# tnestmeyer/reflectance-filtering

Hardware: AMD Instinct MI355X
Metric: megapixels/sec joint-bilateral sigma_c=20 sigma_s=22 @1080p (higher is better)
Workload: dtype f32

## Files before the change

### reflectance_filtering_amd/csrc/rf_api.hip

```cpp
#include "rf_common.hpp"

#include <atomic>
#include <cstring>

#include "reflectance_filtering_debug.h"

namespace rf {

void jbf_shutdown();
void cnn_shutdown();
void gf_shutdown();

char *last_error_buf()
{
    static thread_local char buf[512] = "";
    return buf;
}

int fail(int code, const char *fmt, ...)
{
    va_list ap;
    va_start(ap, fmt);
    vsnprintf(last_error_buf(), 512, fmt, ap);
    va_end(ap);
    return code;
}

static std::atomic<int> g_debug[kDbgCount];

int debug_get(int id) { return g_debug[id].load(std::memory_order_relaxed); }

}

extern "C" int rf_debug_option(const char *name, int value)
{
    static const char *const names[] = {"gf_two_kernel",     "jbf_stage_only",
                                                      "jbf_compiler_loop", "jbf_tile64_only",
                                                      "jbf_tune",          "jbf_f32_untiled",
                                                      "cnn_lds_columns",   "gf_seg_rows",
                                                      "gf_one_stream",     "gf_force_two_streams",
                                                      "gf_guide_cache",    "gf_chained",        "gf_no_compact",
                                                      "gf_exp_skip",       "gf_stagger",        "gf_parts",
                                                      "gf_s1_cap",         "gf_s1_min_wgs",
                                                      "jbf_lookahead1",    "gf_s1_legacy_strips",
                                                      "gf_exact_all_flagged", "gf_cw_chan_run",   "gf_exact",
                                                      "jbf_no_msad",       "colorize_chunk_px"};
    static_assert(sizeof(names) / sizeof(names[0]) == rf::kDbgCount, "one name per DebugOption");
    if (name)
        for (int i = 0; i < rf::kDbgCount; i++)
            if (std::strcmp(name, names[i]) == 0)
                return rf::g_debug[i].exchange(value < 0 ? 0 : value);
    return rf::fail(RF_E_BADARG, "rf_debug_option: unknown option '%s'", name ? name : "(null)");
}

__global__ void clock_probe_kernel(unsigned long long *out, unsigned long long ticks)
{
    if (threadIdx.x != 0)
        return;
    const unsigned long long r0 = __builtin_amdgcn_s_memrealtime();
    const unsigned long long c0 = __builtin_amdgcn_s_memtime();
    unsigned long long r1 = r0;
    while (r1 - r0 < ticks) {
        __builtin_amdgcn_s_sleep(64);
        r1 = __builtin_amdgcn_s_memrealtime();
    }
    const unsigned long long c1 = __builtin_amdgcn_s_memtime();
    r1 = __builtin_amdgcn_s_memrealtime();
    out[0] = c1 - c0;
    out[1] = r1 - r0;
}

extern "C" int rf_debug_clock_probe(unsigned long long *out2, int micros, void *stream)
{
    if (!out2 || micros < 1 || micros > 1000000)
        return rf::fail(RF_E_BADARG, "rf_debug_clock_probe: bad argument");
    hipLaunchKernelGGL(clock_probe_kernel, dim3(1), dim3(64), 0, (hipStream_t)stream, out2,
                       (unsigned long long)micros * 100ull);
    RF_HIP_CHECK(hipGetLastError());
    return RF_OK;
}

#ifdef RF_GF_DEV_ONLY
extern "C" int rf_version(void) { return RF_VERSION | 0x40000000; }
#else
extern "C" int rf_version(void) { return RF_VERSION; }
#endif

#ifndef RF_TOOLCHAIN
#define RF_TOOLCHAIN "unknown toolchain"
#endif
extern "C" const char *rf_debug_build_info(void) { return RF_TOOLCHAIN; }

extern "C" const char *rf_last_error(void) { return rf::last_error_buf(); }

extern "C" int rf_shutdown(void)
{
    rf::jbf_shutdown();
    rf::cnn_shutdown();
    rf::gf_shutdown();
// ... 3 lines not shown
```

### reflectance_filtering_amd/csrc/rf_common.hpp

```cpp
#pragma once
#include <hip/hip_runtime.h>

#include <cstdarg>
#include <cstdint>
#include <cstdio>

#include "reflectance_filtering.h"

namespace rf {

char *last_error_buf();
int fail(int code, const char *fmt, ...);

#define RF_HIP_CHECK(expr)                                                                   \
    do {                                                                                     \
        hipError_t _e = (expr);                                                              \
        if (_e != hipSuccess)                                                                \
            return ::rf::fail(RF_E_HIP, "%s failed: %s (%s:%d)", #expr, hipGetErrorString(_e), \
                              __FILE__, __LINE__);                                           \
    } while (0)

__host__ __device__ inline int border_interpolate(int p, int len, int border)
{
    if ((unsigned)p < (unsigned)len)
// ... 22 lines not shown
__device__ inline uint8_t saturate_u8(float v)
{
    if (!(fabsf(v) < 2147483648.0f))
        return 0;
    int iv = __float2int_rn(v);
    iv = iv < 0 ? 0 : (iv > 255 ? 255 : iv);
    return (uint8_t)iv;
}

inline int ceil_div(int a, int b) { return (a + b - 1) / b; }

inline bool ranges_overlap(const void *a, size_t na, const void *b, size_t nb)
{
    const uintptr_t a0 = (uintptr_t)a, b0 = (uintptr_t)b;
    return a0 < b0 + nb && b0 < a0 + na;
}

inline bool stream_is_capturing(hipStream_t stream)
{
    hipStreamCaptureStatus cs = hipStreamCaptureStatusNone;
    if (hipStreamIsCapturing(stream, &cs) != hipSuccess) {
        (void)hipGetLastError();
        return false;
    }
    return cs != hipStreamCaptureStatusNone;
}

enum DebugOption {
    kDbgGfTwoKernel = 0,
    kDbgJbfStageOnly,
    kDbgJbfCompilerLoop,
    kDbgJbfTile64Only,
    kDbgJbfTune,
    kDbgJbfF32Untiled,
    kDbgCnnLdsColumns,
    kDbgGfSegRows,
    kDbgGfOneStream,
    kDbgGfForceTwoStreams,
    kDbgGfGuideCache,
    kDbgGfChained,
    kDbgGfNoCompact,
    kDbgGfExpSkip,
    kDbgGfStagger,
    kDbgGfParts,
    kDbgGfS1Cap,
    kDbgGfS1MinWgs,
    kDbgJbfLookahead1,
    kDbgGfS1LegacyStrips,
    kDbgGfExactAllFlagged,
    kDbgGfCwChanRun,
    kDbgGfExact,
    kDbgJbfNoMsad,
    kDbgColorizeChunkPx,
    kDbgCount
};
int debug_get(int id);

}
```

### reflectance_filtering_amd/csrc/rf_jbf.hip

```cpp
#include <algorithm>
#include <mutex>
#include <vector>

#include "rf_jbf_common.hpp"
#include "rf_jbf_tables.hpp"
#include "rf_jbf_taploops.hpp"

namespace rf {
namespace {

constexpr int kTileW = 64;
constexpr int kMaxLds = 160 * 1024;
constexpr int kTlw2 = 144;
constexpr int kJbfMaxTiledR4 = 468;
constexpr int kJbfStageOnly = 0x1000, kJbfCompilerLoop = 0x2000, kJbfTile64Only = 0x4000;
constexpr int kJbfLookahead1 = 0x8000;
constexpr int kJbfNoMsad = 0x10000;

int jbf_debug_flags()
{
    return (debug_get(kDbgJbfStageOnly) ? kJbfStageOnly : 0) |
           (debug_get(kDbgJbfCompilerLoop) ? kJbfCompilerLoop : 0) |
           (debug_get(kDbgJbfTile64Only) ? kJbfTile64Only : 0) |
           (debug_get(kDbgJbfLookahead1) ? kJbfLookahead1 : 0) |
// ... 212 lines not shown
        const int X = 4 * tx + p + r4;
        jc[p] = tile[(ty + radius) * TLW + (X & 3) * Q4 + (X >> 2)].x;
    }
    const uint32_t lut_lane_addr = lds_addr(lutrep) + lane_lut * 4u;
    const uint32_t sw_addr0 = lds_addr(swl);
    const uint32_t tile_lane_addr = lds_addr(tile) + (uint32_t)tx * 8u;

    float sum[kPix][SCN];
    float wsum[kPix];
#pragma unroll
    for (int p = 0; p < kPix; p++) {
        wsum[p] = 0.f;
#pragma unroll
        for (int c = 0; c < SCN; c++)
            sum[p][c] = 0.f;
    }
    if (SCN == 3 && !all_grey) {
        jbf_tap_loop<SCN, LUTREP, CLAMP, TLW, 8>(lut_lane_addr, sw_addr0, tile_lane_addr, 0u, jc, amax,
                                              ty, radius, r4, sw_len, hwtab, sum, wsum);
    } else {
        float sum1[kPix][1];
#pragma unroll
        for (int p = 0; p < kPix; p++)
            sum1[p][0] = 0.f;
        jbf_tap_loop<1, LUTREP, CLAMP, TLW, 8>(lut_lane_addr, sw_addr0, tile_lane_addr, 0u, jc, amax, ty,
                                            radius, r4, sw_len, hwtab, sum1, wsum);
#pragma unroll
        for (int p = 0; p < kPix; p++)
#pragma unroll
            for (int c = 0; c < SCN; c++)
                sum[p][c] = sum1[p][0];
    }

    store_quad<SCN, SCN>(dst, img, tile_y0 + ty, tile_x0 + 4 * tx, h, w, sum, wsum, flags);
}

constexpr int kT64Lds = 163840;

struct alignas(16) JbfTileRec {
    unsigned long long first;
    int h, w, tile_y0, tile_x0, pad[2];
};
static_assert(sizeof(JbfTileRec) == 32, "the workspace holds 32 bytes per tile");

template <bool kRagged>
struct JbfTilesArg {
    using type = int;
};
template <>
struct JbfTilesArg<true> {
    using type = const JbfTileRec *__restrict__;
};

template <int SCN, int GREP, int CREP, int TLW, int TH = 64, bool kRagged = false>
__global__ __launch_bounds__(1024) void jbf_tile64_kernel(
    const uint8_t *__restrict__ joint, const uint8_t *__restrict__ src, uint8_t *__restrict__ dst,
    int h, int w, int jcn, int radius, int border, const float *__restrict__ lut, int nz,
    const int *__restrict__ hwtab, const float *__restrict__ swsym, int sw_len,
    typename JbfTilesArg<kRagged>::type tiles_x, int tiles_per_img, int flags, int crows, int y_base,
    int x_base)
{
    constexpr int NT = 1024;
    constexpr int QW = NT / TH;
    constexpr int TW = 4 * QW;
    static_assert(TH == 64 || TH == 32 || ((TH == 16 || TH == 128) && SCN == 1), "tile shapes");
    static_assert(QW >= 32 || (QW == 16 && TLW % 32 == 16) || (QW == 8 && TLW % 32 == 8),
                  "row pitch keeps the rows of a half-wave on disjoint banks");
    constexpr int Q4 = TLW / 4;
    extern __shared__ __align__(16) unsigned char smem[];
    volatile int *flag_word = reinterpret_cast<volatile int *>(smem);
    const bool need_sw = (flags & (kJbfCompilerLoop | kJbfLookahead1)) != 0;
    float *swl = reinterpret_cast<float *>(smem + 16);
    const int sw_bytes = need_sw ? ((radius + 1) * sw_len * 4 + 15) & ~15 : 0;
    unsigned char *tile_raw = smem + 16 + sw_bytes;
    if (threadIdx.x == 0)
        *flag_word = 3;
    __syncthreads();

    const int tid = threadIdx.x;
    const int tile_id = xcd_contiguous_tile((int)blockIdx.x, (int)gridDim.x);
    int tile_y0, tile_x0;
    size_t img;
    if constexpr (kRagged) {
        const JbfTileRec *rec = tiles_x + tile_id;
        img = (size_t)rec->first;
        h = rec->h;
        w = rec->w;
        tile_y0 = rec->tile_y0;
        tile_x0 = rec->tile_x0;
    } else {
        const int img_idx = tile_id / tiles_per_img;
        const int t_in_img = tile_id - img_idx * tiles_per_img;
        tile_y0 = y_base + (t_in_img / tiles_x) * TH;
        tile_x0 = x_base + (t_in_img % tiles_x) * TW;
        img = (size_t)img_idx * h * w;
    }
    const int r4 = (radius + 3) & ~3;
    const int tx = tid % QW;
    const int ty = tid / QW;

    if (need_sw)
        for (int i = tid; i < (radius + 1) * sw_len; i += NT)
            swl[i] = swsym[i];
    float *lut_g = reinterpret_cast<float *>(smem + kT64Lds - nz * GREP * 4);
    for (int i = tid; i < nz * GREP; i += NT)
        lut_g[i] = lut[i / GREP];
    uint32_t *tile4 = reinterpret_cast<uint32_t *>(tile_raw);
    int grey = 1, grey_joint = 1;
    const bool j1_ok = !(flags & kJbfCompilerLoop);
    const bool j1 = SCN == 1 && jcn != 3 && j1_ok;
    const uint32_t j1_scale = (uint32_t)(jcn == 1 ? 1 : 3) * (GREP * 4u);
    const int tlh = TH + 2 * radius;
    for (int item = tid; item < tlh * Q4; item += NT) {
        const int ry = item / Q4, k = item - ry * Q4;
        const int gy = border_interpolate(tile_y0 - radius + ry, h, border);
        uint32_t jv[4], sv[4];
        load_tile_quad(joint, src, img, gy, tile_x0 - r4 + 4 * k, w, jcn, SCN, border, jv, sv);
#pragma unroll
        for (int u = 0; u < 4; u++) {
            if (SCN == 3)
                grey &= (int)(((sv[u] ^ (sv[u] >> 8)) & 0xffffu) == 0u);
            if (jcn == 3)
                grey_joint &= (int)(((jv[u] ^ (jv[u] >> 8)) & 0xffffu) == 0u);
            const uint32_t jfield = j1 ? (jv[u] & 0xffu) * j1_scale : jv[u];
            tile4[ry * TLW + u * Q4 + k] = jfield | (sv[u] << 24);
        }
    }
    const int grey_bits = block_all2(grey, grey_joint, const_cast<int *>(flag_word));
    const int all_grey = grey_bits & 1;
    if (flags & kJbfStageOnly)
        return;
    const bool j1_late = !j1 && j1_ok && (SCN == 1 || all_grey) && (grey_bits & 2);
    if (j1_late) {
        for (int idx = tid; idx < tlh * TLW; idx += NT) {
            const uint32_t t = tile4[idx];
            tile4[idx] = (t & 0xffu) * j1_scale | (t & 0xff000000u);
        }
        __syncthreads();
    }

    const uint32_t sw_addr0 = lds_addr(swl);
    if (SCN == 1 || all_grey) {
        uint32_t jc[kPix];
#pragma unroll
        for (int p = 0; p < kPix; p++) {
            const int X = 4 * tx + p + r4;
            jc[p] = tile4[(ty + radius) * TLW + (X & 3) * Q4 + (X >> 2)] & 0x00ffffffu;
        }
        float sum1[kPix][1], wsum[kPix];
#pragma unroll
        for (int p = 0; p < kPix; p++) {
            sum1[p][0] = 0.f;
            wsum[p] = 0.f;
        }
        const uint32_t lut_lane_addr = lds_addr(lut_g) + (uint32_t)(tid & (GREP - 1)) * 4u;
        const uint32_t tile_lane_addr = lds_addr(tile4) + (uint32_t)tx * 4u;
        if (flags & kJbfCompilerLoop)
            jbf_tap_loop<1, GREP, false, TLW, 4>(lut_lane_addr, sw_addr0, tile_lane_addr, 0u, jc, 0u,
                                                 ty, radius, r4, sw_len, hwtab, sum1, wsum);
        else if (flags & kJbfLookahead1) {
            if (j1 || j1_late)
                jbf_tap_loop_grey4<GREP, TLW, true>(lut_lane_addr, sw_addr0, tile_lane_addr, jc, ty,
                                                    radius, r4, sw_len, hwtab, sum1, wsum);
            else
                jbf_tap_loop_grey4<GREP, TLW>(lut_lane_addr, sw_addr0, tile_lane_addr, jc, ty, radius,
                                              r4, sw_len, hwtab, sum1, wsum);
        } else if (j1 || j1_late)
            jbf_tap_loop_grey4_la2<GREP, TLW, true>(lut_lane_addr, swsym, tile_lane_addr, jc, ty,
                                                    radius, r4, sw_len, hwtab, sum1, wsum);
        else if (!(flags & kJbfNoMsad) && jbf_wave_takes_msad(jc))
            jbf_tap_loop_grey4_la2<GREP, TLW, false, false, true>(lut_lane_addr, swsym, tile_lane_addr, jc,
                                                                  ty, radius, r4, sw_len, hwtab, sum1, wsum);
        else
            jbf_tap_loop_grey4_la2<GREP, TLW>(lut_lane_addr, swsym, tile_lane_addr, jc, ty, radius,
                                              r4, sw_len, hwtab, sum1, wsum);
        store_quad<1, SCN>(dst, img, tile_y0 + ty, tile_x0 + 4 * tx, h, w, sum1, wsum, flags);
        return;
    }

    if constexpr (SCN == 3) {
        if (crows == TH) {
            uint16_t *plane_b = reinterpret_cast<uint16_t *>(tile_raw + (size_t)tlh * TLW * 4);
            float *lut_c = reinterpret_cast<float *>(smem + kT64Lds - nz * CREP * 4);
            __syncthreads();
            for (int i = tid; i < nz * CREP; i += NT)
                lut_c[i] = lut[i / CREP];
            for (int item = tid; item < tlh * Q4; item += NT) {
                const int ry = item / Q4, k = item - ry * Q4;
                const int gy = border_interpolate(tile_y0 - radius + ry, h, border);
                uint32_t jv[4], sv[4];
                load_tile_quad(joint, src, img, gy, tile_x0 - r4 + 4 * k, w, jcn, 3, border, jv, sv);
#pragma unroll
                for (int u = 0; u < 4; u++)
                    plane_b[ry * TLW + u * Q4 + k] = (uint16_t)(sv[u] >> 8);
            }
            __syncthreads();
            uint32_t jc[kPix];
#pragma unroll
            for (int p = 0; p < kPix; p++) {
                const int X = 4 * tx + p + r4;
                jc[p] = tile4[(ty + radius) * TLW + (X & 3) * Q4 + (X >> 2)] & 0x00ffffffu;
            }
            float sum[kPix][3], wsum[kPix];
#pragma unroll
            for (int p = 0; p < kPix; p++) {
                wsum[p] = 0.f;
                sum[p][0] = sum[p][1] = sum[p][2] = 0.f;
            }
            const uint32_t lut_lane_addr = lds_addr(lut_c) + (uint32_t)(tid & (CREP - 1)) * 4u;
            if (flags & kJbfCompilerLoop)
                jbf_tap_loop<3, CREP, false, TLW, 6>(lut_lane_addr, sw_addr0,
                                                     lds_addr(tile4) + (uint32_t)tx * 4u,
                                                     lds_addr(plane_b) + (uint32_t)tx * 2u, jc, 0u,
                                                     ty, radius, r4, sw_len, hwtab, sum, wsum);
            else if (!(flags & kJbfNoMsad) && jbf_wave_takes_msad(jc))
                jbf_tap_loop_rgb6<CREP, TLW, false, true>(lut_lane_addr, swsym,
                                                          lds_addr(tile4) + (uint32_t)tx * 4u,
                                                          lds_addr(plane_b) + (uint32_t)tx * 2u, jc, ty,
                                                          radius, r4, sw_len, hwtab, sum, wsum);
            else
                jbf_tap_loop_rgb6<CREP, TLW>(lut_lane_addr, swsym,
                                             lds_addr(tile4) + (uint32_t)tx * 4u,
                                             lds_addr(plane_b) + (uint32_t)tx * 2u, jc, ty, radius,
                                             r4, sw_len, hwtab, sum, wsum);
            store_quad<3, 3>(dst, img, tile_y0 + ty, tile_x0 + 4 * tx, h, w, sum, wsum, flags);
            return;
        }
        if constexpr (TH != 64)
            return;
        float *lut_c = reinterpret_cast<float *>(smem + kT64Lds - nz * CREP * 4);
        const int tlh8 = crows + 2 * radius;
        uint16_t *plane_b = reinterpret_cast<uint16_t *>(tile_raw + (size_t)tlh8 * TLW * 4);
        for (int half = 0; half * crows < 64; half++) {
            const int y0 = tile_y0 + crows * half;
            if (y0 >= h)
                break;
            __syncthreads();
            if (half == 0)
                for (int i = tid; i < nz * CREP; i += NT)
                    lut_c[i] = lut[i / CREP];
            for (int item = tid; item < tlh8 * Q4; item += NT) {
                const int ry = item / Q4, k = item - ry * Q4;
                const int gy = border_interpolate(y0 - radius + ry, h, border);
                uint32_t jv[4], sv[4];
                load_tile_quad(joint, src, img, gy, tile_x0 - r4 + 4 * k, w, jcn, 3, border, jv, sv);
#pragma unroll
                for (int u = 0; u < 4; u++) {
                    tile4[ry * TLW + u * Q4 + k] = jv[u] | (sv[u] << 24);
                    plane_b[ry * TLW + u * Q4 + k] = (uint16_t)(sv[u] >> 8);
                }
            }
            __syncthreads();
            if (tid < 16 * crows) {
                uint32_t jc[kPix];
#pragma unroll
                for (int p = 0; p < kPix; p++) {
                    const int X = 4 * tx + p + r4;
                    jc[p] = tile4[(ty + radius) * TLW + (X & 3) * Q4 + (X >> 2)] & 0x00ffffffu;
                }
                float sum[kPix][3], wsum[kPix];
#pragma unroll
                for (int p = 0; p < kPix; p++) {
                    wsum[p] = 0.f;
                    sum[p][0] = sum[p][1] = sum[p][2] = 0.f;
                }
                const uint32_t lut_lane_addr = lds_addr(lut_c) + (uint32_t)(tid & (CREP - 1)) * 4u;
                if (flags & kJbfCompilerLoop)
                    jbf_tap_loop<3, CREP, false, TLW, 6>(lut_lane_addr, sw_addr0,
                                                         lds_addr(tile4) + (uint32_t)tx * 4u,
                                                         lds_addr(plane_b) + (uint32_t)tx * 2u, jc, 0u,
                                                         ty, radius, r4, sw_len, hwtab, sum, wsum);
                else if (!(flags & kJbfNoMsad) && jbf_wave_takes_msad(jc))
                    jbf_tap_loop_rgb6<CREP, TLW, false, true>(lut_lane_addr, swsym,
                                                              lds_addr(tile4) + (uint32_t)tx * 4u,
                                                              lds_addr(plane_b) + (uint32_t)tx * 2u, jc,
                                                              ty, radius, r4, sw_len, hwtab, sum, wsum);
                else
                    jbf_tap_loop_rgb6<CREP, TLW>(lut_lane_addr, swsym,
                                                 lds_addr(tile4) + (uint32_t)tx * 4u,
                                                 lds_addr(plane_b) + (uint32_t)tx * 2u, jc, ty, radius,
                                                 r4, sw_len, hwtab, sum, wsum);
                store_quad<3, 3>(dst, img, y0 + ty, tile_x0 + 4 * tx, h, w, sum, wsum, flags);
            }
        }
    }
}

__device__ inline void store_quad_channel(uint8_t *dst, size_t img, int oy, int ox0, int h, int w,
                                          int c, const float (&sum)[kPix][1],
                                          const float (&wsum)[kPix], int flags)
{
    if (oy >= h || ox0 >= w)
        return;
    uint8_t *o = dst + (img + (size_t)oy * w + ox0) * 3 + c;
#pragma unroll
    for (int p = 0; p < kPix; p++) {
        if (ox0 + p >= w)
            break;
        const float d = (flags & RF_JBF_TRUE_DIVISION) ? wsum[p] : __fdiv_rn(1.0f, wsum[p]);
        o[p * 3] = saturate_u8(finish_value(sum[p][0], d, flags));
    }
}

__global__ void lds_oob_probe_kernel(uint32_t *out)
{
    extern __shared__ __align__(16) unsigned char smem[];
    uint32_t *w = reinterpret_cast<uint32_t *>(smem);
    for (int i = threadIdx.x; i < kT64Lds / 4; i += blockDim.x)
        w[i] = 0xdeadbeefu;
    __syncthreads();
    uint32_t bad = 0;
    const uint32_t addrs[4] = {(uint32_t)kT64Lds + 4u * threadIdx.x, (uint32_t)kT64Lds + 61056u,
                               262140u, (uint32_t)kT64Lds - 4u};
#pragma unroll
    for (int k = 0; k < 4; k++) {
        uint32_t v;
        asm volatile("ds_read_b32 %0, %1\n s_waitcnt lgkmcnt(0)" : "=v"(v) : "v"(addrs[k]));
        bad |= (k < 3) ? (v != 0u) : (v != 0xdeadbeefu);
    }
    if (bad)
        atomicOr(out, 1u);
}

struct Tiled2Config {
    int th, lutrep;
    bool full_lut;
};

size_t tiled2_lds_bytes(const JbfTables &t, int th, int lutrep, bool full_lut)
{
    const int lut_len = full_lut ? 256 * t.joint_cn : t.lut_len;
    const size_t lut_bytes = ((size_t)lut_len * lutrep * 4 + 15) & ~(size_t)15;
    const size_t sw_bytes = ((size_t)(t.radius + 1) * t.sw_len * 4 + 15) & ~(size_t)15;
    return 16 + lut_bytes + sw_bytes + (size_t)kTlw2 * (th + 2 * t.radius) * sizeof(uint2);
}

template <int SCN, int TH, int LUTREP>
int launch_tiled2(const JbfTables &t, bool full_lut, const uint8_t *joint, const uint8_t *src,
// ... 30 lines not shown
        if (g_oob_ok[dev] >= 0) {
            *ok = g_oob_ok[dev] == 1;
            return RF_OK;
        }
    }
    CaptureRelax relax;
    uint32_t *d_flag = nullptr;
    hipStream_t ps = nullptr;
    RF_HIP_CHECK(hipStreamCreateWithFlags(&ps, hipStreamNonBlocking));
    struct StreamGuard {
        hipStream_t s;
        ~StreamGuard() { (void)hipStreamDestroy(s); }
    } guard{ps};
    RF_HIP_CHECK(hipMalloc(&d_flag, sizeof(uint32_t)));
    RF_HIP_CHECK(hipMemsetAsync(d_flag, 0, sizeof(uint32_t), ps));
    RF_HIP_CHECK(hipFuncSetAttribute((const void *)lds_oob_probe_kernel,
                                     hipFuncAttributeMaxDynamicSharedMemorySize, kT64Lds));
    hipLaunchKernelGGL(lds_oob_probe_kernel, dim3(8), dim3(256), kT64Lds, ps, d_flag);
    uint32_t flag = 1;
    RF_HIP_CHECK(hipMemcpyAsync(&flag, d_flag, sizeof(flag), hipMemcpyDeviceToHost, ps));
    RF_HIP_CHECK(hipStreamSynchronize(ps));
    (void)hipFree(d_flag);
    std::lock_guard<std::mutex> lock(g_oob_mu);
    g_oob_ok[dev] = flag == 0 ? 1 : 0;
    *ok = flag == 0;
    return RF_OK;
}

int tile64_fits(const JbfTables &t, int nz, int grep, int crep, int scn, int tlw, int th, int flags)
{
    if (2 * t.r4 + 4 * (1024 / th) + 8 > tlw)
        return 0;
    const bool need_sw = (flags & (kJbfCompilerLoop | kJbfLookahead1)) != 0;
    const size_t sw_bytes =
        16 + (need_sw ? ((size_t)(t.radius + 1) * t.sw_len * 4 + 15) & ~(size_t)15 : 0);
    const size_t grey = sw_bytes + (size_t)tlw * (th + 2 * t.radius) * 4 + (size_t)nz * grep * 4;
    if (grey > (size_t)kT64Lds)
        return 0;
    if (scn == 1)
        return 32;
    if (sw_bytes + (size_t)tlw * (th + 2 * t.radius) * 6 + (size_t)nz * crep * 4 <= (size_t)kT64Lds)
        return th;
    if (th != 64)
        return 0;
    for (int crows = 32; crows >= 8; crows >>= 1) {
        const size_t col =
            sw_bytes + (size_t)tlw * (crows + 2 * t.radius) * 6 + (size_t)nz * crep * 4;
        if (col <= (size_t)kT64Lds)
            return crows;
    }
    return 0;
}

template <int SCN, int GREP, int CREP, int TLW, int TH = 64>
int launch_tile64(const JbfTables &t, int nz, int crows, const uint8_t *joint, const uint8_t *src,
                  uint8_t *dst, int n, int h, int w, int jcn, int border, int flags,
                  hipStream_t stream, int y_base = 0, int rows = -1, int x_base = 0, int cols = -1)
{
    if (rows < 0)
        rows = h;
    if (cols < 0)
        cols = w;
    const int tiles_x = ceil_div(cols, 4 * (1024 / TH)), tiles_y = ceil_div(rows, TH);
    const long long blocks = (long long)tiles_x * tiles_y * n;
    if (blocks > 0x7fffffffLL)
        return fail(RF_E_UNSUPPORTED, "rf_jbf_u8: batch too large for one launch");
    auto kern = jbf_tile64_kernel<SCN, GREP, CREP, TLW, TH>;
    RF_HIP_CHECK(hipFuncSetAttribute((const void *)kern, hipFuncAttributeMaxDynamicSharedMemorySize,
                                     kT64Lds));
    hipLaunchKernelGGL(kern, dim3((unsigned)blocks), dim3(1024), kT64Lds, stream, joint, src, dst,
                       h, w, jcn, t.radius, border, t.d_lut, nz, t.d_hw, t.d_swsym, t.sw_len,
                       tiles_x, tiles_x * tiles_y, flags, crows, y_base, x_base);
    return RF_OK;
}

struct Tile64Areas {
    int rows_main, cols_main, s32, s16, sx;
};

Tile64Areas tile64_areas(const JbfTables &t, int nz, int grep, int crep, int scn, int flags, int h,
                         int w)
{
    const bool only64 = (flags & kJbfTile64Only) != 0;
    int sx = 0;
    if (scn == 1 && !only64 && (w & 63) > 0 && (w & 63) <= 32 &&
        tile64_fits(t, nz, grep, crep, scn, 136, 128, flags) > 0 && ceil_div(h, 128) < ceil_div(h, 64))
        sx = w & 63;
    const int cols_main = w - sx;
    const int rem = h & 63;
    const bool ok32 = tile64_fits(t, nz, grep, crep, scn, 208, 32, flags) > 0;
    const bool ok16 = scn == 1 && tile64_fits(t, nz, grep, crep, scn, 336, 16, flags) > 0;
    int s32 = 0, s16 = 0;
    if (rem > 0 && rem <= 16 && ok16)
        s16 = rem;
    else if (rem > 0 && rem <= 32 && ok32)
        s32 = rem;
    else if (rem > 32 && rem <= 48 && ok32 && ok16)
        s32 = 32, s16 = rem - 32;
    const int strip_blocks =
        (s32 ? ceil_div(cols_main, 128) : 0) + (s16 ? ceil_div(cols_main, 256) : 0);
    if (only64 || cols_main == 0 || ((s32 || s16) && strip_blocks >= ceil_div(cols_main, 64)))
        s32 = s16 = 0;
    return Tile64Areas{h - s32 - s16, cols_main, s32, s16, sx};
}

template <int SCN, int GREP, int CREP>
int launch_tile64_rows(const JbfTables &t, int nz, int crows, const uint8_t *joint,
                       const uint8_t *src, uint8_t *dst, int n, int h, int w, int jcn, int border,
                       int flags, hipStream_t stream)
{
    const Tile64Areas a = tile64_areas(t, nz, GREP, CREP, SCN, flags, h, w);
    const int rows_main = a.rows_main, cols_main = a.cols_main, s32 = a.s32, s16 = a.s16, sx = a.sx;
    int rc = RF_OK;
    if (rows_main > 0 && cols_main > 0)
        rc = launch_tile64<SCN, GREP, CREP, 144>(t, nz, crows, joint, src, dst, n, h, w, jcn,
                                                 border, flags, stream, 0, rows_main, 0, cols_main);
    if (rc == RF_OK && s32)
        rc = launch_tile64<SCN, GREP, CREP, 208, 32>(t, nz, 32, joint, src, dst, n, h, w, jcn,
                                                     border, flags, stream, rows_main, s32, 0,
                                                     cols_main);
    if constexpr (SCN == 1) {
        if (rc == RF_OK && s16)
            rc = launch_tile64<1, GREP, CREP, 336, 16>(t, nz, 32, joint, src, dst, n, h, w, jcn,
                                                       border, flags, stream, rows_main + s32, s16,
                                                       0, cols_main);
// ... 39 lines not shown
    bool tiled = false;
    bool slab = false;
    Tile64Shape shape{};
    SlabShape slab_shape{};
    std::vector<JbfTileRec> recs[kRaggedClasses];
};

void plan_ragged(const JbfTables &t, int n, const int *heights, const int *widths, int src_cn,
                 int flags, int tune, RaggedPlan *plan)
{
    const int nz = t.lut_len < 256 * t.joint_cn ? t.lut_len - 1 : t.lut_len;
    if ((flags & RF_JBF_FORCE_GENERIC) || tune != 0)
        return;
    plan->tiled = tile64_choose(t, nz, src_cn, flags, &plan->shape);
    plan->slab = !plan->tiled && slab_choose(t, nz, src_cn, &plan->slab_shape);
    if (!plan->tiled && !plan->slab)
        return;
    const Tile64Shape &s = plan->shape;
    unsigned long long first = 0;
    for (int i = 0; i < n; i++) {
        const int h = heights[i], w = widths[i];
        Tile64Areas a{h, w, 0, 0, 0};
        if (plan->tiled && s.tlw == 144)
            a = tile64_areas(t, nz, s.grep, s.crep, src_cn, flags, h, w);
        const int area[kRaggedClasses][4] = {{0, a.rows_main, 0, a.cols_main},
                                             {a.rows_main, a.s32, 0, a.cols_main},
                                             {a.rows_main + a.s32, a.s16, 0, a.cols_main},
                                             {0, a.sx ? h : 0, a.cols_main, a.sx}};
        for (int c = 0; c < kRaggedClasses; c++) {
            const int th = kRaggedTh[c], tw = 4096 / th;
            for (int y = 0; y < area[c][1]; y += th)
                for (int x = 0; x < area[c][3]; x += tw)
                    plan->recs[c].push_back(
                        JbfTileRec{first, h, w, area[c][0] + y, area[c][2] + x, {0, 0}});
        }
        first += (unsigned long long)h * w;
    }
}

template <int SCN, int GREP, int CREP, int TLW, int TH>
int launch_tile64_ragged(const JbfTables &t, int nz, int crows, const uint8_t *joint,
                         const uint8_t *src, uint8_t *dst, const JbfTileRec *d_recs, size_t ntiles,
                         int jcn, int border, int flags, hipStream_t stream)
{
    if (ntiles == 0)
        return RF_OK;
    if (ntiles > (size_t)0x7fffffff)
        return fail(RF_E_UNSUPPORTED, "rf_jbf_ragged_u8: too many tiles for one launch");
    auto kern = jbf_tile64_kernel<SCN, GREP, CREP, TLW, TH, true>;
    RF_HIP_CHECK(hipFuncSetAttribute((const void *)kern, hipFuncAttributeMaxDynamicSharedMemorySize,
                                     kT64Lds));
    hipLaunchKernelGGL(kern, dim3((unsigned)ntiles), dim3(1024), kT64Lds, stream, joint, src, dst, 0,
                       0, jcn, t.radius, border, t.d_lut, nz, t.d_hw, t.d_swsym, t.sw_len, d_recs, 0,
                       flags, crows, 0, 0);
    return RF_OK;
}

template <int SCN, int GREP, int CREP, int TLW>
int launch_ragged(const JbfTables &t, int nz, const RaggedPlan &plan, const uint8_t *joint,
                  const uint8_t *src, uint8_t *dst, const JbfTileRec *const *d_recs, int jcn,
                  int border, int flags, hipStream_t stream)
{
    int rc = launch_tile64_ragged<SCN, GREP, CREP, TLW, 64>(t, nz, plan.shape.crows, joint, src, dst,
                                                            d_recs[0], plan.recs[0].size(), jcn,
                                                            border, flags, stream);
    if constexpr (TLW == 144) {
        if (rc == RF_OK)
            rc = launch_tile64_ragged<SCN, GREP, CREP, 208, 32>(t, nz, 32, joint, src, dst, d_recs[1],
                                                                plan.recs[1].size(), jcn, border,
                                                                flags, stream);
        if constexpr (SCN == 1) {
            if (rc == RF_OK)
                rc = launch_tile64_ragged<1, GREP, CREP, 336, 16>(t, nz, 32, joint, src, dst,
                                                                  d_recs[2], plan.recs[2].size(), jcn,
                                                                  border, flags, stream);
            if (rc == RF_OK)
                rc = launch_tile64_ragged<1, GREP, CREP, 136, 128>(t, nz, 32, joint, src, dst,
                                                                   d_recs[3], plan.recs[3].size(),
                                                                   jcn, border, flags, stream);
        }
    }
    return rc;
}

template <int GREP, int TLW, bool kRagged = false>
__global__ __launch_bounds__(1024) void jbf_slab_kernel(
    const uint8_t *__restrict__ joint, const uint8_t *__restrict__ src, uint8_t *__restrict__ dst,
    int h, int w, int jcn, int scn, int radius, int border, const float *__restrict__ lut, int nz,
    const int *__restrict__ hwtab, const float *__restrict__ swsym, int sw_len,
    typename JbfTilesArg<kRagged>::type tiles_x, int tiles_per_img, int flags, int crows_g, int slab_g,
    int crows_c, int slab_c)
{
    constexpr int NT = 1024, Q4 = TLW / 4, QW = 16;
    static_assert(TLW % 32 == 16, "row pitch keeps the rows of a half-wave on disjoint banks");
    extern __shared__ __align__(16) unsigned char smem[];
    int *flag_word = reinterpret_cast<int *>(smem);
    uint32_t *tile4 = reinterpret_cast<uint32_t *>(smem + 16);
    const int tid = threadIdx.x;
    if (tid == 0)
        *flag_word = 3;
    const int tile_id = xcd_contiguous_tile((int)blockIdx.x, (int)gridDim.x);
    int tile_y0, tile_x0;
    size_t img;
    if constexpr (kRagged) {
        const JbfTileRec *rec = tiles_x + tile_id;
        img = (size_t)rec->first;
        h = rec->h;
// ... 538 lines not shown
```

Baseline: 2489.

## Add persistent-grid form of the 64-row JBF tile kernel sized to CU count

The uniform 64x64 tiled joint-bilateral kernel can now run as a persistent kernel: the grid is capped at the CU count rounded down to a multiple of 8, and each workgroup loops over tiles with a grid stride. The LUT and spatial-weight staging into LDS happens once per workgroup instead of once per tile, and a double-buffered flag word avoids races between iterations. The aim is to cut per-workgroup launch and LUT setup cost, at the price of possible tail imbalance, since one 1024-thread workgroup per CU may leave occupancy and latency hiding lower than with a full grid.

```diff
diff --git a/reflectance_filtering_amd/csrc/rf_api.hip b/reflectance_filtering_amd/csrc/rf_api.hip
--- a/reflectance_filtering_amd/csrc/rf_api.hip
+++ b/reflectance_filtering_amd/csrc/rf_api.hip
@@ -44,7 +44,8 @@
                                                       "gf_s1_cap",         "gf_s1_min_wgs",
                                                       "jbf_lookahead1",    "gf_s1_legacy_strips",
                                                       "gf_exact_all_flagged", "gf_cw_chan_run",   "gf_exact",
-                                                      "jbf_no_msad",       "colorize_chunk_px"};
+                                                      "jbf_no_msad",       "colorize_chunk_px",
+                                                      "jbf_no_persist",    "jbf_persist_grid"};
     static_assert(sizeof(names) / sizeof(names[0]) == rf::kDbgCount, "one name per DebugOption");
     if (name)
         for (int i = 0; i < rf::kDbgCount; i++)
diff --git a/reflectance_filtering_amd/csrc/rf_common.hpp b/reflectance_filtering_amd/csrc/rf_common.hpp
--- a/reflectance_filtering_amd/csrc/rf_common.hpp
+++ b/reflectance_filtering_amd/csrc/rf_common.hpp
@@ -98,6 +98,8 @@
     kDbgGfExact,
     kDbgJbfNoMsad,
     kDbgColorizeChunkPx,
+    kDbgJbfNoPersist,
+    kDbgJbfPersistGrid,
     kDbgCount
 };
 int debug_get(int id);
diff --git a/reflectance_filtering_amd/csrc/rf_jbf.hip b/reflectance_filtering_amd/csrc/rf_jbf.hip
--- a/reflectance_filtering_amd/csrc/rf_jbf.hip
+++ b/reflectance_filtering_amd/csrc/rf_jbf.hip
@@ -288,14 +288,40 @@
     using type = const JbfTileRec *__restrict__;
 };
 
-template <int SCN, int GREP, int CREP, int TLW, int TH = 64, bool kRagged = false>
+struct JbfNoCount {
+};
+template <bool kPersist>
+struct JbfCountArg {
+    using type = JbfNoCount;
+};
+template <>
+struct JbfCountArg<true> {
+    using type = int;
+};
+
+__device__ inline bool jbf_next_tile(int &launch_idx, int ntiles)
+{
+    launch_idx += (int)gridDim.x;
+    return launch_idx < ntiles;
+}
+__device__ inline bool jbf_next_tile(int &, JbfNoCount) { return false; }
+
+template <int SCN, int GREP, int CREP, int TLW, int TH = 64, bool kRagged = false, bool kPersist = false>
 __global__ __launch_bounds__(1024) void jbf_tile64_kernel(
     const uint8_t *__restrict__ joint, const uint8_t *__restrict__ src, uint8_t *__restrict__ dst,
     int h, int w, int jcn, int radius, int border, const float *__restrict__ lut, int nz,
     const int *__restrict__ hwtab, const float *__restrict__ swsym, int sw_len,
     typename JbfTilesArg<kRagged>::type tiles_x, int tiles_per_img, int flags, int crows, int y_base,
-    int x_base)
-{
+    int x_base, typename JbfCountArg<kPersist>::type ntiles)
+{
+    static_assert(!kPersist || (!kRagged && TH == 64), "the persistent form serves the uniform 64x64 area");
+#define RF_JBF_TILE_DONE                                                                          \
+    {                                                                                             \
+        if constexpr (kPersist)                                                                   \
+            continue;                                                                             \
+        else                                                                                      \
+            return;                                                                               \
+    }
     constexpr int NT = 1024;
     constexpr int QW = NT / TH;
     constexpr int TW = 4 * QW;
@@ -304,190 +330,161 @@
                   "row pitch keeps the rows of a half-wave on disjoint banks");
     constexpr int Q4 = TLW / 4;
     extern __shared__ __align__(16) unsigned char smem[];
-    volatile int *flag_word = reinterpret_cast<volatile int *>(smem);
-    const bool need_sw = (flags & (kJbfCompilerLoop | kJbfLookahead1)) != 0;
-    float *swl = reinterpret_cast<float *>(smem + 16);
-    const int sw_bytes = need_sw ? ((radius + 1) * sw_len * 4 + 15) & ~15 : 0;
-    unsigned char *tile_raw = smem + 16 + sw_bytes;
-    if (threadIdx.x == 0)
-        *flag_word = 3;
-    __syncthreads();
-
-    const int tid = threadIdx.x;
-    const int tile_id = xcd_contiguous_tile((int)blockIdx.x, (int)gridDim.x);
-    int tile_y0, tile_x0;
-    size_t img;
-    if constexpr (kRagged) {
-        const JbfTileRec *rec = tiles_x + tile_id;
-        img = (size_t)rec->first;
-        h = rec->h;
-        w = rec->w;
-        tile_y0 = rec->tile_y0;
-        tile_x0 = rec->tile_x0;
-    } else {
-        const int img_idx = tile_id / tiles_per_img;
-        const int t_in_img = tile_id - img_idx * tiles_per_img;
-        tile_y0 = y_base + (t_in_img / tiles_x) * TH;
-        tile_x0 = x_base + (t_in_img % tiles_x) * TW;
-        img = (size_t)img_idx * h * w;
-    }
-    const int r4 = (radius + 3) & ~3;
-    const int tx = tid % QW;
-    const int ty = tid / QW;
-
-    if (need_sw)
-        for (int i = tid; i < (radius + 1) * sw_len; i += NT)
-            swl[i] = swsym[i];
-    float *lut_g = reinterpret_cast<float *>(smem + kT64Lds - nz * GREP * 4);
-    for (int i = tid; i < nz * GREP; i += NT)
-        lut_g[i] = lut[i / GREP];
-    uint32_t *tile4 = reinterpret_cast<uint32_t *>(tile_raw);
-    int grey = 1, grey_joint = 1;
-    const bool j1_ok = !(flags & kJbfCompilerLoop);
-    const bool j1 = SCN == 1 && jcn != 3 && j1_ok;
-    const uint32_t j1_scale = (uint32_t)(jcn == 1 ? 1 : 3) * (GREP * 4u);
-    const int tlh = TH + 2 * radius;
-    for (int item = tid; item < tlh * Q4; item += NT) {
-        const int ry = item / Q4, k = item - ry * Q4;
-        const int gy = border_interpolate(tile_y0 - radius + ry, h, border);
-        uint32_t jv[4], sv[4];
-        load_tile_quad(joint, src, img, gy, tile_x0 - r4 + 4 * k, w, jcn, SCN, border, jv, sv);
-#pragma unroll
-        for (int u = 0; u < 4; u++) {
-            if (SCN == 3)
-                grey &= (int)(((sv[u] ^ (sv[u] >> 8)) & 0xffffu) == 0u);
-            if (jcn == 3)
-                grey_joint &= (int)(((jv[u] ^ (jv[u] >> 8)) & 0xffffu) == 0u);
-            const uint32_t jfield = j1 ? (jv[u] & 0xffu) * j1_scale : jv[u];
-            tile4[ry * TLW + u * Q4 + k] = jfield | (sv[u] << 24);
-        }
-    }
-    const int grey_bits = block_all2(grey, grey_joint, const_cast<int *>(flag_word));
-    const int all_grey = grey_bits & 1;
-    if (flags & kJbfStageOnly)
-        return;
-    const bool j1_late = !j1 && j1_ok && (SCN == 1 || all_grey) && (grey_bits & 2);
-    if (j1_late) {
-        for (int idx = tid; idx < tlh * TLW; idx += NT) {
-            const uint32_t t = tile4[idx];
-            tile4[idx] = (t & 0xffu) * j1_scale | (t & 0xff000000u);
-        }
+    int lut_now = GREP;
+    int launch_idx = (int)blockIdx.x, trip = 0;
+    if constexpr (kPersist) {
+        if (flags & (kJbfCompilerLoop | kJbfLookahead1))
+            for (int i = (int)threadIdx.x; i < (radius + 1) * sw_len; i += NT)
+                reinterpret_cast<float *>(smem + 16)[i] = swsym[i];
+        for (int i = (int)threadIdx.x; i < nz * GREP; i += NT)
+            reinterpret_cast<float *>(smem + kT64Lds - nz * GREP * 4)[i] = lut[i / GREP];
+    }
+    do {
+        volatile int *flag_word = reinterpret_cast<volatile int *>(smem) + (kPersist ? trip & 1 : 0);
+        trip ^= 1;
+        const bool need_sw = (flags & (kJbfCompilerLoop | kJbfLookahead1)) != 0;
+        float *swl = reinterpret_cast<float *>(smem + 16);
+        const int sw_bytes = need_sw ? ((radius + 1) * sw_len * 4 + 15) & ~15 : 0;
+        unsigned char *tile_raw = smem + 16 + sw_bytes;
+        if (threadIdx.x == 0)
+            *flag_word = 3;
         __syncthreads();
-    }
-
-    const uint32_t sw_addr0 = lds_addr(swl);
-    if (SCN == 1 || all_grey) {
-        uint32_t jc[kPix];
-#pragma unroll
-        for (int p = 0; p < kPix; p++) {
-            const int X = 4 * tx + p + r4;
-            jc[p] = tile4[(ty + radius) * TLW + (X & 3) * Q4 + (X >> 2)] & 0x00ffffffu;
-        }
-        float sum1[kPix][1], wsum[kPix];
-#pragma unroll
-        for (int p = 0; p < kPix; p++) {
-            sum1[p][0] = 0.f;
-            wsum[p] = 0.f;
-        }
-        const uint32_t lut_lane_addr = lds_addr(lut_g) + (uint32_t)(tid & (GREP - 1)) * 4u;
-        const uint32_t tile_lane_addr = lds_addr(tile4) + (uint32_t)tx * 4u;
-        if (flags & kJbfCompilerLoop)
-            jbf_tap_loop<1, GREP, false, TLW, 4>(lut_lane_addr, sw_addr0, tile_lane_addr, 0u, jc, 0u,
-                                                 ty, radius, r4, sw_len, hwtab, sum1, wsum);
-        else if (flags & kJbfLookahead1) {
-            if (j1 || j1_late)
-                jbf_tap_loop_grey4<GREP, TLW, true>(lut_lane_addr, sw_addr0, tile_lane_addr, jc, ty,
-                                                    radius, r4, sw_len, hwtab, sum1, wsum);
-            else
-                jbf_tap_loop_grey4<GREP, TLW>(lut_lane_addr, sw_addr0, tile_lane_addr, jc, ty, radius,
-                                              r4, sw_len, hwtab, sum1, wsum);
-        } else if (j1 || j1_late)
-            jbf_tap_loop_grey4_la2<GREP, TLW, true>(lut_lane_addr, swsym, tile_lane_addr, jc, ty,
-                                                    radius, r4, sw_len, hwtab, sum1, wsum);
-        else if (!(flags & kJbfNoMsad) && jbf_wave_takes_msad(jc))
-            jbf_tap_loop_grey4_la2<GREP, TLW, false, false, true>(lut_lane_addr, swsym, tile_lane_addr, jc,
-                                                                  ty, radius, r4, sw_len, hwtab, sum1, wsum);
+
+        const int tid = threadIdx.x;
+        int tile_id;
+        if constexpr (kPersist)
+            tile_id = xcd_contiguous_tile(launch_idx, ntiles);
         else
-            jbf_tap_loop_grey4_la2<GREP, TLW>(lut_lane_addr, swsym, tile_lane_addr, jc, ty, radius,
-                                              r4, sw_len, hwtab, sum1, wsum);
-        store_quad<1, SCN>(dst, img, tile_y0 + ty, tile_x0 + 4 * tx, h, w, sum1, wsum, flags);
-        return;
-    }
-
-    if constexpr (SCN == 3) {
-        if (crows == TH) {
-            uint16_t *plane_b = reinterpret_cast<uint16_t *>(tile_raw + (size_t)tlh * TLW * 4);
-            float *lut_c = reinterpret_cast<float *>(smem + kT64Lds - nz * CREP * 4);
-            __syncthreads();
-            for (int i = tid; i < nz * CREP; i += NT)
-                lut_c[i] = lut[i / CREP];
-            for (int item = tid; item < tlh * Q4; item += NT) {
-                const int ry = item / Q4, k = item - ry * Q4;
-                const int gy = border_interpolate(tile_y0 - radius + ry, h, border);
-                uint32_t jv[4], sv[4];
-                load_tile_quad(joint, src, img, gy, tile_x0 - r4 + 4 * k, w, jcn, 3, border, jv, sv);
-#pragma unroll
-                for (int u = 0; u < 4; u++)
-                    plane_b[ry * TLW + u * Q4 + k] = (uint16_t)(sv[u] >> 8);
+            tile_id = xcd_contiguous_tile((int)blockIdx.x, (int)gridDim.x);
+        int tile_y0, tile_x0;
+        size_t img;
+        if constexpr (kRagged) {
+            const JbfTileRec *rec = tiles_x + tile_id;
+            img = (size_t)rec->first;
+            h = rec->h;
+            w = rec->w;
+            tile_y0 = rec->tile_y0;
+            tile_x0 = rec->tile_x0;
+        } else {
+            const int img_idx = tile_id / tiles_per_img;
+            const int t_in_img = tile_id - img_idx * tiles_per_img;
+            tile_y0 = y_base + (t_in_img / tiles_x) * TH;
+            tile_x0 = x_base + (t_in_img % tiles_x) * TW;
+            img = (size_t)img_idx * h * w;
+        }
+        const int r4 = (radius + 3) & ~3;
+        const int tx = tid % QW;
+        const int ty = tid / QW;
+
+        if constexpr (!kPersist)
+            if (need_sw)
+                for (int i = tid; i < (radius + 1) * sw_len; i += NT)
+                    swl[i] = swsym[i];
+        float *lut_g = reinterpret_cast<float *>(smem + kT64Lds - nz * GREP * 4);
+        if constexpr (!kPersist)
+            for (int i = tid; i < nz * GREP; i += NT)
+                lut_g[i] = lut[i / GREP];
+        uint32_t *tile4 = reinterpret_cast<uint32_t *>(tile_raw);
+        int grey = 1, grey_joint = 1;
+        const bool j1_ok = !(flags & kJbfCompilerLoop);
+        const bool j1 = SCN == 1 && jcn != 3 && j1_ok;
+        const uint32_t j1_scale = (uint32_t)(jcn == 1 ? 1 : 3) * (GREP * 4u);
+        const int tlh = TH + 2 * radius;
+        for (int item = tid; item < tlh * Q4; item += NT) {
+            const int ry = item / Q4, k = item - ry * Q4;
+            const int gy = border_interpolate(tile_y0 - radius + ry, h, border);
+            uint32_t jv[4], sv[4];
+            load_tile_quad(joint, src, img, gy, tile_x0 - r4 + 4 * k, w, jcn, SCN, border, jv, sv);
+#pragma unroll
+            for (int u = 0; u < 4; u++) {
+                if (SCN == 3)
+                    grey &= (int)(((sv[u] ^ (sv[u] >> 8)) & 0xffffu) == 0u);
+                if (jcn == 3)
+                    grey_joint &= (int)(((jv[u] ^ (jv[u] >> 8)) & 0xffffu) == 0u);
+                const uint32_t jfield = j1 ? (jv[u] & 0xffu) * j1_scale : jv[u];
+                tile4[ry * TLW + u * Q4 + k] = jfield | (sv[u] << 24);
+            }
+        }
+        const int grey_bits = block_all2(grey, grey_joint, const_cast<int *>(flag_word));
+        const int all_grey = grey_bits & 1;
+        if (flags & kJbfStageOnly)
+            RF_JBF_TILE_DONE;
+        if constexpr (kPersist && SCN == 3 && GREP != CREP) {
+            if (all_grey && lut_now != GREP) {
+                for (int i = tid; i < nz * GREP; i += NT)
+                    lut_g[i] = lut[i / GREP];
+                lut_now = GREP;
+                __syncthreads();
+            }
+        }
+        const bool j1_late = !j1 && j1_ok && (SCN == 1 || all_grey) && (grey_bits & 2);
+        if (j1_late) {
+            for (int idx = tid; idx < tlh * TLW; idx += NT) {
+                const uint32_t t = tile4[idx];
+                tile4[idx] = (t & 0xffu) * j1_scale | (t & 0xff000000u);
             }
             __syncthreads();
+        }
+
+        const uint32_t sw_addr0 = lds_addr(swl);
+        if (SCN == 1 || all_grey) {
             uint32_t jc[kPix];
 #pragma unroll
             for (int p = 0; p < kPix; p++) {
                 const int X = 4 * tx + p + r4;
                 jc[p] = tile4[(ty + radius) * TLW + (X & 3) * Q4 + (X >> 2)] & 0x00ffffffu;
             }
-            float sum[kPix][3], wsum[kPix];
+            float sum1[kPix][1], wsum[kPix];
 #pragma unroll
             for (int p = 0; p < kPix; p++) {
+                sum1[p][0] = 0.f;
                 wsum[p] = 0.f;
-                sum[p][0] = sum[p][1] = sum[p][2] = 0.f;
             }
-            const uint32_t lut_lane_addr = lds_addr(lut_c) + (uint32_t)(tid & (CREP - 1)) * 4u;
+            const uint32_t lut_lane_addr = lds_addr(lut_g) + (uint32_t)(tid & (GREP - 1)) * 4u;
+            const uint32_t tile_lane_addr = lds_addr(tile4) + (uint32_t)tx * 4u;
             if (flags & kJbfCompilerLoop)
-                jbf_tap_loop<3, CREP, false, TLW, 6>(lut_lane_addr, sw_addr0,
-                                                     lds_addr(tile4) + (uint32_t)tx * 4u,
-                                                     lds_addr(plane_b) + (uint32_t)tx * 2u, jc, 0u,
-                                                     ty, radius, r4, sw_len, hwtab, sum, wsum);
+                jbf_tap_loop<1, GREP, false, TLW, 4>(lut_lane_addr, sw_addr0, tile_lane_addr, 0u, jc, 0u,
+                                                     ty, radius, r4, sw_len, hwtab, sum1, wsum);
+            else if (flags & kJbfLookahead1) {
+                if (j1 || j1_late)
+                    jbf_tap_loop_grey4<GREP, TLW, true>(lut_lane_addr, sw_addr0, tile_lane_addr, jc, ty,
+                                                        radius, r4, sw_len, hwtab, sum1, wsum);
+                else
+                    jbf_tap_loop_grey4<GREP, TLW>(lut_lane_addr, sw_addr0, tile_lane_addr, jc, ty, radius,
+                                                  r4, sw_len, hwtab, sum1, wsum);
+            } else if (j1 || j1_late)
+                jbf_tap_loop_grey4_la2<GREP, TLW, true>(lut_lane_addr, swsym, tile_lane_addr, jc, ty,
+                                                        radius, r4, sw_len, hwtab, sum1, wsum);
             else if (!(flags & kJbfNoMsad) && jbf_wave_takes_msad(jc))
-                jbf_tap_loop_rgb6<CREP, TLW, false, true>(lut_lane_addr, swsym,
-                                                          lds_addr(tile4) + (uint32_t)tx * 4u,
-                                                          lds_addr(plane_b) + (uint32_t)tx * 2u, jc, ty,
-                                                          radius, r4, sw_len, hwtab, sum, wsum);
+                jbf_tap_loop_grey4_la2<GREP, TLW, false, false, true>(lut_lane_addr, swsym, tile_lane_addr, jc,
+                                                                      ty, radius, r4, sw_len, hwtab, sum1, wsum);
             else
-                jbf_tap_loop_rgb6<CREP, TLW>(lut_lane_addr, swsym,
-                                             lds_addr(tile4) + (uint32_t)tx * 4u,
-                                             lds_addr(plane_b) + (uint32_t)tx * 2u, jc, ty, radius,
-                                             r4, sw_len, hwtab, sum, wsum);
-            store_quad<3, 3>(dst, img, tile_y0 + ty, tile_x0 + 4 * tx, h, w, sum, wsum, flags);
-            return;
-        }
-        if constexpr (TH != 64)
-            return;
-        float *lut_c = reinterpret_cast<float *>(smem + kT64Lds - nz * CREP * 4);
-        const int tlh8 = crows + 2 * radius;
-        uint16_t *plane_b = reinterpret_cast<uint16_t *>(tile_raw + (size_t)tlh8 * TLW * 4);
-        for (int half = 0; half * crows < 64; half++) {
-            const int y0 = tile_y0 + crows * half;
-            if (y0 >= h)
-                break;
-            __syncthreads();
-            if (half == 0)
-                for (int i = tid; i < nz * CREP; i += NT)
-                    lut_c[i] = lut[i / CREP];
-            for (int item = tid; item < tlh8 * Q4; item += NT) {
-                const int ry = item / Q4, k = item - ry * Q4;
-                const int gy = border_interpolate(y0 - radius + ry, h, border);
-                uint32_t jv[4], sv[4];
-                load_tile_quad(joint, src, img, gy, tile_x0 - r4 + 4 * k, w, jcn, 3, border, jv, sv);
-#pragma unroll
-                for (int u = 0; u < 4; u++) {
-                    tile4[ry * TLW + u * Q4 + k] = jv[u] | (sv[u] << 24);
-                    plane_b[ry * TLW + u * Q4 + k] = (uint16_t)(sv[u] >> 8);
+                jbf_tap_loop_grey4_la2<GREP, TLW>(lut_lane_addr, swsym, tile_lane_addr, jc, ty, radius,
+                                                  r4, sw_len, hwtab, sum1, wsum);
+            store_quad<1, SCN>(dst, img, tile_y0 + ty, tile_x0 + 4 * tx, h, w, sum1, wsum, flags);
+            RF_JBF_TILE_DONE;
+        }
+
+        if constexpr (SCN == 3) {
+            if (crows == TH) {
+                uint16_t *plane_b = reinterpret_cast<uint16_t *>(tile_raw + (size_t)tlh * TLW * 4);
+                float *lut_c = reinterpret_cast<float *>(smem + kT64Lds - nz * CREP * 4);
+                if (!kPersist || lut_now != CREP) {
+                    __syncthreads();
+                    for (int i = tid; i < nz * CREP; i += NT)
+                        lut_c[i] = lut[i / CREP];
+                    lut_now = CREP;
                 }
-            }
-            __syncthreads();
-            if (tid < 16 * crows) {
+                for (int item = tid; item < tlh * Q4; item += NT) {
+                    const int ry = item / Q4, k = item - ry * Q4;
+                    const int gy = border_interpolate(tile_y0 - radius + ry, h, border);
+                    uint32_t jv[4], sv[4];
+                    load_tile_quad(joint, src, img, gy, tile_x0 - r4 + 4 * k, w, jcn, 3, border, jv, sv);
+#pragma unroll
+                    for (int u = 0; u < 4; u++)
+                        plane_b[ry * TLW + u * Q4 + k] = (uint16_t)(sv[u] >> 8);
+                }
+                __syncthreads();
                 uint32_t jc[kPix];
 #pragma unroll
                 for (int p = 0; p < kPix; p++) {
@@ -509,17 +506,78 @@
                 else if (!(flags & kJbfNoMsad) && jbf_wave_takes_msad(jc))
                     jbf_tap_loop_rgb6<CREP, TLW, false, true>(lut_lane_addr, swsym,
                                                               lds_addr(tile4) + (uint32_t)tx * 4u,
-                                                              lds_addr(plane_b) + (uint32_t)tx * 2u, jc,
-                                                              ty, radius, r4, sw_len, hwtab, sum, wsum);
+                                                              lds_addr(plane_b) + (uint32_t)tx * 2u, jc, ty,
+                                                              radius, r4, sw_len, hwtab, sum, wsum);
                 else
                     jbf_tap_loop_rgb6<CREP, TLW>(lut_lane_addr, swsym,
                                                  lds_addr(tile4) + (uint32_t)tx * 4u,
                                                  lds_addr(plane_b) + (uint32_t)tx * 2u, jc, ty, radius,
                                                  r4, sw_len, hwtab, sum, wsum);
-                store_quad<3, 3>(dst, img, y0 + ty, tile_x0 + 4 * tx, h, w, sum, wsum, flags);
+                store_quad<3, 3>(dst, img, tile_y0 + ty, tile_x0 + 4 * tx, h, w, sum, wsum, flags);
+                RF_JBF_TILE_DONE;
             }
-        }
-    }
+            if constexpr (TH != 64)
+                return;
+            float *lut_c = reinterpret_cast<float *>(smem + kT64Lds - nz * CREP * 4);
+            const int tlh8 = crows + 2 * radius;
+            uint16_t *plane_b = reinterpret_cast<uint16_t *>(tile_raw + (size_t)tlh8 * TLW * 4);
+            for (int half = 0; half * crows < 64; half++) {
+                const int y0 = tile_y0 + crows * half;
+                if (y0 >= h)
+                    break;
+                __syncthreads();
+                if (half == 0 && (!kPersist || lut_now != CREP)) {
+                    for (int i = tid; i < nz * CREP; i += NT)
+                        lut_c[i] = lut[i / CREP];
+                    lut_now = CREP;
+                }
+                for (int item = tid; item < tlh8 * Q4; item += NT) {
+                    const int ry = item / Q4, k = item - ry * Q4;
+                    const int gy = border_interpolate(y0 - radius + ry, h, border);
+                    uint32_t jv[4], sv[4];
+                    load_tile_quad(joint, src, img, gy, tile_x0 - r4 + 4 * k, w, jcn, 3, border, jv, sv);
+#pragma unroll
+                    for (int u = 0; u < 4; u++) {
+                        tile4[ry * TLW + u * Q4 + k] = jv[u] | (sv[u] << 24);
+                        plane_b[ry * TLW + u * Q4 + k] = (uint16_t)(sv[u] >> 8);
+                    }
+                }
+                __syncthreads();
+                if (tid < 16 * crows) {
+                    uint32_t jc[kPix];
+#pragma unroll
+                    for (int p = 0; p < kPix; p++) {
+                        const int X = 4 * tx + p + r4;
+                        jc[p] = tile4[(ty + radius) * TLW + (X & 3) * Q4 + (X >> 2)] & 0x00ffffffu;
+                    }
+                    float sum[kPix][3], wsum[kPix];
+#pragma unroll
+                    for (int p = 0; p < kPix; p++) {
+                        wsum[p] = 0.f;
+                        sum[p][0] = sum[p][1] = sum[p][2] = 0.f;
+                    }
+                    const uint32_t lut_lane_addr = lds_addr(lut_c) + (uint32_t)(tid & (CREP - 1)) * 4u;
+                    if (flags & kJbfCompilerLoop)
+                        jbf_tap_loop<3, CREP, false, TLW, 6>(lut_lane_addr, sw_addr0,
+                                                             lds_addr(tile4) + (uint32_t)tx * 4u,
+                                                             lds_addr(plane_b) + (uint32_t)tx * 2u, jc, 0u,
+                                                             ty, radius, r4, sw_len, hwtab, sum, wsum);
+                    else if (!(flags & kJbfNoMsad) && jbf_wave_takes_msad(jc))
+                        jbf_tap_loop_rgb6<CREP, TLW, false, true>(lut_lane_addr, swsym,
+                                                                  lds_addr(tile4) + (uint32_t)tx * 4u,
+                                                                  lds_addr(plane_b) + (uint32_t)tx * 2u, jc,
+                                                                  ty, radius, r4, sw_len, hwtab, sum, wsum);
+                    else
+                        jbf_tap_loop_rgb6<CREP, TLW>(lut_lane_addr, swsym,
+                                                     lds_addr(tile4) + (uint32_t)tx * 4u,
+                                                     lds_addr(plane_b) + (uint32_t)tx * 2u, jc, ty, radius,
+                                                     r4, sw_len, hwtab, sum, wsum);
+                    store_quad<3, 3>(dst, img, y0 + ty, tile_x0 + 4 * tx, h, w, sum, wsum, flags);
+                }
+            }
+        }
+    } while (jbf_next_tile(launch_idx, ntiles));
+#undef RF_JBF_TILE_DONE
 }
 
 __device__ inline void store_quad_channel(uint8_t *dst, size_t img, int oy, int ox0, int h, int w,
@@ -656,6 +714,40 @@
     return 0;
 }
 
+std::mutex g_cus_mu;
+std::vector<int> g_cus;
+
+int jbf_persist_grid(int dev, long long tiles, int *grid)
+{
+    *grid = 0;
+    if (debug_get(kDbgJbfNoPersist) || tiles <= 0 || tiles > 0x7fffffffLL - 65536)
+        return RF_OK;
+    const int forced = debug_get(kDbgJbfPersistGrid);
+    if (forced > 0) {
+        if ((forced >= 8 && (forced & 7)) || forced > 65536)
+            return fail(RF_E_BADARG, "jbf_persist_grid: %d is neither a multiple of 8 up to 65536 nor below 8",
+                        forced);
+        *grid = (int)std::min<long long>(forced, tiles);
+        return RF_OK;
+    }
+    int cus = 0;
+    {
+        std::lock_guard<std::mutex> lock(g_cus_mu);
+        if ((int)g_cus.size() <= dev)
+            g_cus.resize(dev + 1, 0);
+        if (g_cus[dev] == 0) {
+            RF_HIP_CHECK(hipDeviceGetAttribute(&g_cus[dev], hipDeviceAttributeMultiprocessorCount, dev));
+            if (g_cus[dev] <= 0)
+                g_cus[dev] = -1;
+        }
+        cus = g_cus[dev];
+    }
+    const int g = cus & ~7;
+    if (g > 0 && tiles > g)
+        *grid = g;
+    return RF_OK;
+}
+
 template <int SCN, int GREP, int CREP, int TLW, int TH = 64>
 int launch_tile64(const JbfTables &t, int nz, int crows, const uint8_t *joint, const uint8_t *src,
                   uint8_t *dst, int n, int h, int w, int jcn, int border, int flags,
@@ -669,12 +761,27 @@
     const long long blocks = (long long)tiles_x * tiles_y * n;
     if (blocks > 0x7fffffffLL)
         return fail(RF_E_UNSUPPORTED, "rf_jbf_u8: batch too large for one launch");
+    if constexpr (TH == 64) {
+        int grid = 0;
+        if (int rc = jbf_persist_grid(t.device, blocks, &grid))
+            return rc;
+        if (grid > 0) {
+            auto pkern = jbf_tile64_kernel<SCN, GREP, CREP, TLW, 64, false, true>;
+            RF_HIP_CHECK(hipFuncSetAttribute((const void *)pkern,
+                                             hipFuncAttributeMaxDynamicSharedMemorySize, kT64Lds));
+            hipLaunchKernelGGL(pkern, dim3((unsigned)grid), dim3(1024), kT64Lds, stream, joint, src,
+                               dst, h, w, jcn, t.radius, border, t.d_lut, nz, t.d_hw, t.d_swsym,
+                               t.sw_len, tiles_x, tiles_x * tiles_y, flags, crows, y_base, x_base,
+                               (int)blocks);
+            return RF_OK;
+        }
+    }
     auto kern = jbf_tile64_kernel<SCN, GREP, CREP, TLW, TH>;
     RF_HIP_CHECK(hipFuncSetAttribute((const void *)kern, hipFuncAttributeMaxDynamicSharedMemorySize,
                                      kT64Lds));
     hipLaunchKernelGGL(kern, dim3((unsigned)blocks), dim3(1024), kT64Lds, stream, joint, src, dst,
                        h, w, jcn, t.radius, border, t.d_lut, nz, t.d_hw, t.d_swsym, t.sw_len,
-                       tiles_x, tiles_x * tiles_y, flags, crows, y_base, x_base);
+                       tiles_x, tiles_x * tiles_y, flags, crows, y_base, x_base, JbfNoCount{});
     return RF_OK;
 }
 
@@ -820,7 +927,7 @@
                                      kT64Lds));
     hipLaunchKernelGGL(kern, dim3((unsigned)ntiles), dim3(1024), kT64Lds, stream, joint, src, dst, 0,
                        0, jcn, t.radius, border, t.d_lut, nz, t.d_hw, t.d_swsym, t.sw_len, d_recs, 0,
-                       flags, crows, 0, 0);
+                       flags, crows, 0, 0, JbfNoCount{});
     return RF_OK;
 }
 
```

After: 2493 (median of 6 runs). No clear change (+0.2%).
